# brodbeck-m/dolfinx_eqlb

Hardware: AMD Instinct MI355X
Metric: equilibrated patches/s (fp64) on 1M-tri Poisson k=2; L2 flux-divergence residual (higher is better)
Workload: dtype f64; 1 GPU; Poisson 1000000 triangles per GPU (crossed unit square 500x500), P2 primal, FluxEqlbSE RT2, homogeneous Dirichlet, fp64; headline=True, patches_per_gpu=501001, cells_per_gpu=1000000, nrhs=1, weak_symmetry=False, partition=none, solver=shuffle, scatter=tiled, accumulate=True

## Files before the change

dolfinx_eqlb_amd/csrc/eqlb_device_common.h:

```cpp
#pragma once

#include "eqlb_internal.h"

namespace eqlb
{

__host__ __device__ constexpr int nd_of(int deg) { return (deg + 1) * (deg + 2) / 2; }
__host__ __device__ constexpr int nrt_of(int k) { return k * (k + 2); }
__host__ __device__ constexpr int nq_of(int k) { return k * (k + 1) / 2; }
__host__ __device__ constexpr int binom(int n, int r)
{
  int v = 1;
  for (int i = 0; i < r; ++i)
    v = v * (n - i) / (i + 1);
  return v;
}
__host__ __device__ constexpr double bcoef(int j, int i)
{
  return (i > j) ? 0.0 : ((i % 2 == 0) ? 1.0 : -1.0) * binom(j, i);
}

#ifndef EQLB_WS_PIVOT_RTOL
#define EQLB_WS_PIVOT_RTOL 1e-11
#endif

__device__ __forceinline__ void wave_sync()
{
  __builtin_amdgcn_fence(__ATOMIC_RELEASE, "wavefront");
  __builtin_amdgcn_wave_barrier();
  __builtin_amdgcn_fence(__ATOMIC_ACQUIRE, "wavefront");
}

__device__ __forceinline__ double shfl_d(double v, int src_lane) { return __shfl(v, src_lane, 64); }

__device__ __forceinline__ int tri(int i, int j) { return i * (i + 1) / 2 + j; }

#ifndef EQLB_USE_DPP
#define EQLB_USE_DPP 1
#endif
template <int CTRL>
__device__ __forceinline__ double dpp_d(double v)
{
  int lo = __double2loint(v), hi = __double2hiint(v);
  lo = __builtin_amdgcn_update_dpp(0, lo, CTRL, 0xf, 0xf, true);
  hi = __builtin_amdgcn_update_dpp(0, hi, CTRL, 0xf, 0xf, true);
  return __hiloint2double(hi, lo);
}
template <int P, int OFF>
__device__ __forceinline__ double lane_down_d(double v, int gbase, int sub)
{
  if constexpr (EQLB_USE_DPP && P <= 16)
    return dpp_d<0x110 + OFF>(v);
  else if constexpr (EQLB_USE_DPP && OFF == 1)
    return dpp_d<0x138>(v);
  else
    return __shfl(v, gbase + ((sub >= OFF) ? sub - OFF : sub), 64);
}
template <int P>
__device__ __forceinline__ double lane_up1_d(double v, int gbase, int sub)
{
  if constexpr (EQLB_USE_DPP && P <= 16)
    return dpp_d<0x101>(v);
  else if constexpr (EQLB_USE_DPP)
    return dpp_d<0x130>(v);
  else
    return __shfl(v, gbase + ((sub + 1 < P) ? sub + 1 : sub), 64);
}
#ifndef EQLB_GSUM_SWIZZLE
#define EQLB_GSUM_SWIZZLE 0
#endif
template <int XOR>
__device__ __forceinline__ double swizzle_xor_d(double v)
{
  constexpr int PAT = (XOR << 10) | 0x1f;
  int lo = __double2loint(v), hi = __double2hiint(v);
  lo = __builtin_amdgcn_ds_swizzle(lo, PAT);
  hi = __builtin_amdgcn_ds_swizzle(hi, PAT);
  return __hiloint2double(hi, lo);
}
template <int P>
__device__ __forceinline__ double group_sum_d(double v, int gbase, int sub)
{
  if constexpr (EQLB_GSUM_SWIZZLE && P <= 16)
  {
    v += swizzle_xor_d<1>(v);
    v += swizzle_xor_d<2>(v);
    if constexpr (P >= 8)
      v += swizzle_xor_d<4>(v);
    if constexpr (P >= 16)
      v += swizzle_xor_d<8>(v);
    return v;
  }
  else if constexpr (EQLB_USE_DPP && P <= 16)
  {
    v += dpp_d<0xB1>(v);
    v += dpp_d<0x4E>(v);
    if constexpr (P >= 8)
      v += dpp_d<0x141>(v);
    if constexpr (P >= 16)
      v += dpp_d<0x140>(v);
    return v;
  }
  else
  {
#pragma unroll
    for (int off = 1; off < P; off <<= 1)
      v += __shfl(v, gbase + (sub ^ off), 64);
    return v;
  }
}

#ifndef EQLB_FAST_RCP
#define EQLB_FAST_RCP 1
#endif
__device__ __forceinline__ double rcp_d(double x)
{
#if EQLB_FAST_RCP
  double r = __builtin_amdgcn_rcp(x);
  r = __builtin_fma(__builtin_fma(-x, r, 1.0), r, r);
  r = __builtin_fma(__builtin_fma(-x, r, 1.0), r, r);
  return r;
#else
  return 1.0 / x;
#endif
}
__device__ __forceinline__ double rsqrt_d(double x)
{
#if EQLB_FAST_RCP
  double y = __builtin_amdgcn_rsq(x);
  y = __builtin_fma(y * 0.5, __builtin_fma(-x * y, y, 1.0), y);
  y = __builtin_fma(y * 0.5, __builtin_fma(-x * y, y, 1.0), y);
  return y;
#else
  return 1.0 / sqrt(x);
#endif
}


constexpr int NCOMBO = 12;
__host__ __device__ constexpr int combo_index(int fm, int fp, bool rev)
{
  return (fm * 2 + ((fp < fm) ? fp : fp - 1)) * 2 + (rev ? 1 : 0);
}

#ifndef EQLB_WQ_PAD
#define EQLB_WQ_PAD 0
#endif
template <int K, int DEG, int P>
struct Sizes
{
  static constexpr int KB = K - 1;
  static constexpr int NADD = (K - 1) * (K - 2) / 2;
  static constexpr int NDIV = K * (K + 1) / 2 - 1;
  static constexpr int NRT = nrt_of(K), ND = nd_of(DEG), NQ = nq_of(K);
  static constexpr int NY = 2 * K + NADD;
  static constexpr int NCOL = 2 * K + NDIV;
  static constexpr int NH = 1 + 2 * KB + NADD;
  static constexpr int NTE = NH * (NH + 1) / 2;
  static constexpr int NTES = NTE + (NTE & 1), NCOLS = NCOL + (NCOL & 1);
  static constexpr int DIMMAX = 1 + KB * P + NADD * P;
  static constexpr int TRI = DIMMAX * (DIMMAX + 1) / 2;
  static constexpr int LDS_GROUP = TRI + DIMMAX;
  static constexpr int HROW = ND * NQ + ((ND * NQ) & 1);
  static constexpr int NS = 3 * NRT * NRT, NF = 9 * ND * K, NHT = 3 * HROW, NDT = 6 * ND * NQ;
  static constexpr int NTET = NCOMBO * 3 * NTES, NWQT = NCOMBO * 3 * NH * NCOLS;
  static constexpr int NHB = 9 * K * K;
  static constexpr int NTAB = NF + NHT + NDT + NTET + NWQT + NHB;
  static constexpr int NVT = 3 * NRT * 2, NVQT = NCOMBO * 2 * NH * 3;
  static constexpr int OFF_TE = NS + NF + NHT + NDT, OFF_V = OFF_TE + NTET + NWQT + NHB, OFF_VQ = OFF_V + NVT;
  static constexpr int NHG = HROW, NWG = NCOMBO * NH * ND * 2, NEV = NHG + NWG;
  static constexpr int OFF_HG = OFF_VQ + NVQT;
  static constexpr int NCMB = 3 * NH * NCOLS, NCMBH = NCMB + ((K == 3) ? EQLB_WQ_PAD : 0);
  static constexpr int NWQH = (NCOMBO / 2) * NCMBH, NTAB_HALF = NTAB - NWQT + NWQH;
  static constexpr int NEV_LDS = (K >= 4) ? NHG : NEV;
  static constexpr int lds_doubles(int block, int solver, int mode = 0)
  {
    return NTAB + (mode ? NEV_LDS : 0) + ((K > 1 && solver == 0) ? (block / P) * LDS_GROUP : 0);
  }
  static constexpr int block_of(int solver)
  {
    if (K >= 4 && solver != 0 && P < 32)
      return 256;
    return (P >= 32) ? 64
                     : ((lds_doubles(256, solver) * 8 <= 65536)
                            ? 256
                            : ((lds_doubles(128, solver) * 8 <= 65536) ? 128 : 64));
  }
};


}
```

dolfinx_eqlb_amd/csrc/eqlb_se_kernels.hip:

```cpp
#include "eqlb_device_common.h"
#include "eqlb_tables_gen.h"

#ifndef EQLB_PCR_SELECTS
#define EQLB_PCR_SELECTS 0
#endif

#ifndef EQLB_SE_TEMPLATES_ONLY
#define EQLB_SE_TEMPLATES_ONLY 0
#endif

namespace eqlb
{

#if !EQLB_SE_TEMPLATES_ONLY
size_t table_doubles(int k, int deg)
{
  const int nrt = nrt_of(k), nd = nd_of(deg), nq = nq_of(k);
  const int kb = k - 1, nadd = (k - 1) * (k - 2) / 2, ndiv = k * (k + 1) / 2 - 1;
  const int nh = 1 + 2 * kb + nadd, ncol = 2 * k + ndiv;
  const int hrow = nd * nq + ((nd * nq) & 1);
  const int nte = nh * (nh + 1) / 2;
  return (size_t)3 * nrt * nrt + (size_t)9 * nd * k + (size_t)3 * hrow + (size_t)6 * nd * nq
         + (size_t)NCOMBO * 3 * (nte + (nte & 1)) + (size_t)NCOMBO * 3 * nh * (ncol + (ncol & 1))
         + (size_t)9 * k * k + (size_t)3 * nrt * 2 + (size_t)NCOMBO * 2 * nh * 3
// ... 52 lines not shown
  if (k == 1 && deg == 0)
    fill_tables_t<1, 0>(out);
  else if (k == 2 && deg == 1)
    fill_tables_t<2, 1>(out);
  else if (k == 3 && deg == 2)
    fill_tables_t<3, 2>(out);
  else if (k == 4 && deg == 3)
    fill_tables_t<4, 3>(out);
  else if (k == 2 && deg == 0)
    fill_tables_t<2, 0>(out);
  else if (k == 3 && deg == 1)
    fill_tables_t<3, 1>(out);
  else if (k == 3 && deg == 0)
    fill_tables_t<3, 0>(out);
  else if (k == 4 && deg >= 0 && deg < 3)
  {
    if (fill_tables_k4_lowdeg(deg, out) != 0)
      return EQLB_ERR_UNSUPPORTED;
  }
  else
    return EQLB_ERR_UNSUPPORTED;
  return (out.size() == table_doubles(k, deg)) ? 0 : EQLB_ERR_UNSUPPORTED;
}
#endif

#ifndef EQLB_EV_FMA
#define EQLB_EV_FMA 1
#endif
#ifndef EQLB_LE_FMA
#define EQLB_LE_FMA 1
#endif
#ifndef EQLB_P2_DIV_NODAL
#define EQLB_P2_DIV_NODAL 1
#endif
#ifndef EQLB_CHAIN_PCR
#define EQLB_CHAIN_PCR 1
#endif

template <bool AL>
__device__ __forceinline__ const double* row16(const double* p)
{
  if constexpr (AL)
    return static_cast<const double*>(__builtin_assume_aligned(p, 16));
  else
    return p;
}

template <int N>
__device__ __forceinline__ void ldrow16(const double* p, double (&r)[N])
{
  static_assert(N % 2 == 0, "row length");
  const double2* q = reinterpret_cast<const double2*>(p);
#pragma unroll
  for (int i = 0; i < N / 2; ++i)
  {
    const double2 v = q[i];
    r[2 * i] = v.x;
    r[2 * i + 1] = v.y;
  }
}

#ifndef EQLB_REV_FMA
#define EQLB_REV_FMA 1
#endif
template <int K>
__device__ __forceinline__ void reversal_apply(const double (&x)[K], const double rho, double (&y)[K])
{
#pragma unroll
  for (int j = 0; j < K; ++j)
  {
    double d = 0.0;
    bool any = false;
#pragma unroll
    for (int c = 0; c <= j; ++c)
    {
      const double coef = bcoef(j, c) - ((j == c) ? 1.0 : 0.0);
      if (coef != 0.0)
      {
        d = any ? __builtin_fma(coef, x[c], d) : coef * x[c];
        any = true;
      }
    }
    y[j] = any ? __builtin_fma(rho, d, x[j]) : x[j];
  }
}
template <int K>
__device__ __forceinline__ void reversal_apply_t(const double (&x)[K], const double rho, double (&y)[K])
{
#pragma unroll
  for (int h = 0; h < K; ++h)
  {
    double d = 0.0;
    bool any = false;
#pragma unroll
    for (int j = h; j < K; ++j)
    {
      const double coef = bcoef(j, h) - ((j == h) ? 1.0 : 0.0);
      if (coef != 0.0)
      {
        d = any ? __builtin_fma(coef, x[j], d) : coef * x[j];
        any = true;
      }
    }
    y[h] = any ? __builtin_fma(rho, d, x[h]) : x[h];
  }
}

template <int K, int DEG, int P, int SOLVER, int SCATTER, int BLOCK, int MODE = 0, bool FULL = false, bool INTR = false>
__device__ __forceinline__ void se_patch_body(const SeArgs& a, const int64_t block_id, double* lds,
                                              const bool tables_staged = false,
                                              const int64_t lane_index = -1, double* tile_slots = nullptr)
{
  using Z = Sizes<K, DEG, P>;
  constexpr int KB = Z::KB, NADD = Z::NADD, NDIV = Z::NDIV, NRT = Z::NRT, ND = Z::ND, NQ = Z::NQ;
  constexpr int NCOL = Z::NCOL, NH = Z::NH;

  constexpr bool AL = K == 2 && DEG == 1;
  static_assert(!AL || (Z::NF % 2 == 0 && Z::NHT % 2 == 0 && Z::NDT % 2 == 0 && Z::NTET % 2 == 0
                        && Z::NWQT % 2 == 0 && (ND * K) % 2 == 0 && Z::HROW % 2 == 0
                        && Z::NTES % 2 == 0 && Z::NCOLS % 2 == 0 && Z::NHB % 2 == 0
                        && Z::NHG % 2 == 0),
                "table rows are not 16-byte aligned");
  double* sF = lds;
  double* sH = sF + Z::NF;
  double* sD = sH + Z::NHT;
  double* sTE = sD + Z::NDT;
  constexpr bool HALFWQ = SCATTER == 2 && K == 3;
  double* sWQ = sTE + Z::NTET;
  double* sHB = sWQ + (HALFWQ ? Z::NWQH : Z::NWQT);
  double* sHG = sHB + Z::NHB;
  const double* sWG = (K >= 4) ? a.tables + Z::OFF_HG + Z::NHG : sHG + Z::NHG;
  (void)sWG;
  double* sA = sHB + Z::NHB + (MODE ? Z::NEV_LDS : 0);
  (void)sA;

  int tid_ = threadIdx.x;
#ifndef EQLB_OPAQUE_K3
#define EQLB_OPAQUE_K3 1
#endif
  if constexpr (SCATTER == 2 && (MODE == 1 || (EQLB_OPAQUE_K3 && K >= 3)))
    asm volatile("" : "+v"(tid_));
  const int tid = tid_;
  if (!tables_staged)
  {
    for (int i = tid; i < Z::NTAB; i += BLOCK)
      lds[i] = a.tables[Z::NS + i];
    if constexpr (MODE == 1)
      for (int i = tid; i < Z::NEV_LDS; i += BLOCK)
        sHG[i] = a.tables[Z::OFF_HG + i];
    __syncthreads();
  }

  const int lane = tid & 63;
  const int sub = lane % P;
  const int gbase = lane - sub;
  const int64_t tl = (lane_index >= 0) ? lane_index : block_id * BLOCK + tid;
  const int64_t patch_local = tl / P;
#ifndef EQLB_FULL_SIMPLE
#define EQLB_FULL_SIMPLE 1
#endif
#ifndef EQLB_FULL_SIMPLE_EV
#define EQLB_FULL_SIMPLE_EV 0
#endif
  constexpr bool FULLS = FULL && EQLB_FULL_SIMPLE && (MODE == 0 || K >= 3 || EQLB_FULL_SIMPLE_EV);
  const bool pvalid = FULLS ? true : (patch_local < a.npatch);
  const int64_t slot = a.slot_offset + tl;
  const int64_t patch = a.patch_offset + patch_local;

  const int r = a.rhs;
  int n = 0;
  int32_t cell_raw = -1;
  uint32_t info = 0u;
  uint8_t flag0 = (uint8_t)PFLAG_INTERIOR, flag = (uint8_t)0;
  if (pvalid)
  {
    n = (int)a.pn[patch];
    cell_raw = a.slot_cell[slot];
    info = a.slot_info[slot];
    flag0 = a.pflag[patch];
    flag = a.pflag[(int64_t)r * a.npatch_total + patch];
  }
  if constexpr (FULL)
  {
    n = P;
    flag0 = (uint8_t)PFLAG_INTERIOR;
    flag = (uint8_t)0;
  }
  if constexpr (INTR)
  {
    flag0 = (uint8_t)PFLAG_INTERIOR;
    flag = (uint8_t)0;
  }
  const bool active = FULL ? true : (cell_raw >= 0);
  const int32_t cell = active ? cell_raw : 0;
  const int fm = (info >> INFO_FM_SHIFT) & 3, fp = (info >> INFO_FP_SHIFT) & 3;
  const int ln = (info >> INFO_LN_SHIFT) & 3;
  const bool rev_m = (info & INFO_REV_M) != 0, rev_p = (info & INFO_REV_P) != 0;
  const int ci = active ? combo_index(fm, fp, rev_m) : 0;
  const double rho_m = rev_m ? 1.0 : 0.0, rho_p = rev_p ? 1.0 : 0.0;
  (void)rho_m;
  (void)rho_p;

  double J00 = 1.0, J01 = 0.0, J10 = 0.0, J11 = 1.0;
  double2 gdat[ND];
  double fdat[ND];
#pragma unroll
  for (int i = 0; i < ND; ++i)
  {
    gdat[i] = make_double2(0.0, 0.0);
    fdat[i] = 0.0;
  }
  if (active)
  {
    const double2* Jp = reinterpret_cast<const double2*>(a.cellJ + 4 * (int64_t)cell);
    const double2* gp_ = reinterpret_cast<const double2*>(a.flux_dg + ((int64_t)a.rhs_in * a.ncells + cell) * (ND * 2));
    const double* fp_ = a.rhs_dg + ((int64_t)a.rhs_in * a.ncells + cell) * ND;
    const double2 j0 = Jp[0], j1 = Jp[1];
#pragma unroll
    for (int i = 0; i < ND; ++i)
      gdat[i] = gp_[i];
#pragma unroll
    for (int i = 0; i < ND; ++i)
      fdat[i] = fp_[i];
    J00 = j0.x;
    J01 = j0.y;
    J10 = j1.x;
    J11 = j1.y;
  }
  const double detJ = J00 * J11 - J01 * J10;
  const double sgn = (detJ > 0.0) ? 1.0 : -1.0;
  const double pf_m = (fm == 1) ? sgn : -sgn;
  const double pf_p = (fp == 1) ? sgn : -sgn;

  const bool interior_geo = (flag0 & PFLAG_INTERIOR) != 0;
  const int nf = interior_geo ? n : n + 1;
  const int nn = (n > 0) ? n : 1;
  const int next = FULLS ? ((sub + 1) & (P - 1)) : ((sub + 1 < nn) ? sub + 1 : (interior_geo ? 0 : sub));
  const int prev = FULLS ? ((sub + P - 1) & (P - 1)) : ((sub > 0) ? sub - 1 : (interior_geo ? nn - 1 : 0));
  const bool has_next = active && (interior_geo || sub < n - 1);
  const bool has_prev = active && (interior_geo || sub > 0);
  const int fi_p = FULLS ? next : (interior_geo ? ((sub + 1 < nn) ? sub + 1 : 0) : sub + 1);
  const int dim = pvalid ? 1 + KB * nf + NADD * n : 0;
  (void)dim;

  int status_local = 0;

  {
    const bool bc0 = (flag & PFLAG_BC0) != 0, bcn = (flag & PFLAG_BCN) != 0;
    const bool d_fixed = bc0 || bcn;

    double gm[K], gpv[K], Rq[NQ];
    double LeG[MODE ? NH : 1];
    (void)LeG;
    {
      const double a00 = J11, a01 = -J01, a10 = -J10, a11 = J00;
      const double nmx = (fm == 2) ? 0.0 : -1.0, nmy = (fm == 0) ? -1.0 : ((fm == 1) ? 0.0 : 1.0);
      const double npx = (fp == 2) ? 0.0 : -1.0, npy = (fp == 0) ? -1.0 : ((fp == 1) ? 0.0 : 1.0);
      const double num0 = a00 * nmx + a10 * nmy, num1 = a01 * nmx + a11 * nmy;
      const double nup0 = a00 * npx + a10 * npy, nup1 = a01 * npx + a11 * npy;
#pragma unroll
      for (int j = 0; j < K; ++j)
        gm[j] = gpv[j] = 0.0;
#pragma unroll
      for (int q = 0; q < NQ; ++q)
        Rq[q] = 0.0;
      if constexpr (MODE == 1)
      {
#pragma unroll
        for (int h = 0; h < NH; ++h)
          LeG[h] = 0.0;
        if (active)
        {
          const double* tH = row16<AL>(sH + ln * Z::HROW);
          const double* wg = row16<AL>(sWG + ci * NH * ND * 2);

          const double dh0 = (ln == 0) ? -1.0 : ((ln == 1) ? 1.0 : 0.0);
          const double dh1 = (ln == 0) ? -1.0 : ((ln == 2) ? 1.0 : 0.0);
#pragma unroll
          for (int i = 0; i < ND; ++i)
          {
            const double2 g2 = gdat[i];
            const double fd = detJ * fdat[i];
            const double gg = dh0 * (a00 * g2.x + a01 * g2.y) + dh1 * (a10 * g2.x + a11 * g2.y);
            const double jt0 = J00 * g2.x + J10 * g2.y, jt1 = J01 * g2.x + J11 * g2.y;
#pragma unroll
            for (int q = 0; q < NQ; ++q)
#if EQLB_EV_FMA
              Rq[q] = __builtin_fma(gg, sHG[i * NQ + q], __builtin_fma(fd, tH[i * NQ + q], Rq[q]));
#else
              Rq[q] += fd * tH[i * NQ + q] + gg * sHG[i * NQ + q];
#endif
#pragma unroll
            for (int h = 0; h < NH; ++h)
            {
              if constexpr (AL)
              {
                const double2 w2 = reinterpret_cast<const double2*>(wg)[h * ND + i];
#if EQLB_EV_FMA
                LeG[h] = __builtin_fma(w2.y, jt1, __builtin_fma(w2.x, jt0, LeG[h]));
#else
                LeG[h] += w2.x * jt0 + w2.y * jt1;
#endif
              }
              else
#if EQLB_EV_FMA
                LeG[h] = __builtin_fma(wg[(h * ND + i) * 2 + 1], jt1, __builtin_fma(wg[(h * ND + i) * 2], jt0, LeG[h]));
#else
                LeG[h] += wg[(h * ND + i) * 2] * jt0 + wg[(h * ND + i) * 2 + 1] * jt1;
#endif
            }
          }
        }
      }
      else if (active)
      {
        const double* tF_m = row16<AL>(sF + (fm * 3 + ln) * ND * K);
        const double* tF_p = row16<AL>(sF + (fp * 3 + ln) * ND * K);
        const double* tH = row16<AL>(sH + ln * Z::HROW);
        const double* tD = sD + ln * ND * 2 * NQ;
        double fdv[ND], dvg = 0.0;
        double ax[(DEG == 2) ? ND : 1], by[(DEG == 2) ? ND : 1];
        (void)fdv;
        (void)tD;
        (void)ax;
        (void)by;
#pragma unroll
        for (int i = 0; i < ND; ++i)
        {
          const double2 g2 = gdat[i];
          const double fv = fdat[i];
          const double gnm = g2.x * num0 + g2.y * num1;
          const double gnp = g2.x * nup0 + g2.y * nup1;
          const double gh0 = a00 * g2.x + a01 * g2.y;
          const double gh1 = a10 * g2.x + a11 * g2.y;
          const double fd = detJ * fv;
          if constexpr (AL)
          {
            double rm[K], rp[K];
            ldrow16<K>(tF_m + i * K, rm);
            ldrow16<K>(tF_p + i * K, rp);
#pragma unroll
            for (int j = 0; j < K; ++j)
            {
              gm[j] += rm[j] * gnm;
              gpv[j] += rp[j] * gnp;
            }
          }
          else
          {
#pragma unroll
            for (int j = 0; j < K; ++j)
            {
              gm[j] += tF_m[i * K + j] * gnm;
              gpv[j] += tF_p[i * K + j] * gnp;
            }
          }
          if constexpr (DEG == 1)
          {
            fdv[i] = fd;
            if (i == 0)
              dvg = -(gh0 + gh1);
            else if (i == 1)
              dvg += gh0;
            else
              dvg += gh1;
          }
          else if constexpr (DEG == 0 && K >= 2)
          {
#pragma unroll
            for (int q = 0; q < NQ; ++q)
              Rq[q] = __builtin_fma(fd, tH[q], Rq[q]);
          }
          else if constexpr (DEG == 2 && EQLB_P2_DIV_NODAL)
          {
            fdv[i] = fd;
            ax[i] = gh0;
            by[i] = gh1;
          }
          else
          {
#pragma unroll
            for (int q = 0; q < NQ; ++q)
              Rq[q] = __builtin_fma(-gh1, tD[(i * 2 + 1) * NQ + q],
                                    __builtin_fma(-gh0, tD[(i * 2 + 0) * NQ + q], __builtin_fma(fd, tH[i * NQ + q], Rq[q])));
          }
        }
        if constexpr (DEG == 2 && EQLB_P2_DIV_NODAL)
        {
          double dvn[ND];
          dvn[0] = 4.0 * (ax[5] + by[4]) - 3.0 * (ax[0] + by[0]) - ax[1] - by[2];
          dvn[1] = ax[0] + by[0] + 3.0 * ax[1] - by[2] + 4.0 * (by[3] - by[5] - ax[5]);
          dvn[2] = ax[0] + by[0] - ax[1] + 3.0 * by[2] + 4.0 * (ax[3] - ax[4] - by[4]);
          dvn[3] = 0.5 * (dvn[1] + dvn[2]);
          dvn[4] = 0.5 * (dvn[0] + dvn[2]);
          dvn[5] = 0.5 * (dvn[0] + dvn[1]);
#pragma unroll
          for (int i = 0; i < ND; ++i)
          {
            const double w = fdv[i] - dvn[i];
#pragma unroll
            for (int q = 0; q < NQ; ++q)
              Rq[q] = __builtin_fma(w, tH[i * NQ + q], Rq[q]);
          }
        }
        if constexpr (DEG == 1)
        {
          double rH[Z::HROW];
          if constexpr (AL)
            ldrow16<Z::HROW>(tH, rH);
          else
          {
#pragma unroll
            for (int e = 0; e < ND * NQ; ++e)
              rH[e] = tH[e];
          }
#pragma unroll
          for (int i = 0; i < ND; ++i)
#pragma unroll
            for (int q = 0; q < NQ; ++q)
              Rq[q] += (fdv[i] - dvg) * rH[i * NQ + q];
        }
#pragma unroll
        for (int j = 0; j < K; ++j)
        {
          gm[j] *= pf_m;
          gpv[j] *= pf_p;
        }
      }
    }

    double mu_m[K], mu_p[K];
    {
      double Jv[K];
      {
        double gmn[K];
#pragma unroll
        for (int j = 0; j < K; ++j)
          gmn[j] = shfl_d(gm[j], gbase + next);
#if EQLB_REV_FMA
        double gt[K];
        reversal_apply<K>(gmn, rho_p, gt);
#pragma unroll
        for (int j = 0; j < K; ++j)
          Jv[j] = has_next ? gpv[j] + gt[j] : 0.0;
#else
#pragma unroll
        for (int j = 0; j < K; ++j)
        {
          double t = 0.0;
          if (rev_p)
          {
#pragma unroll
            for (int i = 0; i < K; ++i)
              t += bcoef(j, i) * gmn[i];
          }
          else
            t = gmn[j];
          Jv[j] = has_next ? gpv[j] + t : 0.0;
        }
#endif
      }
      const double Jprev0 = shfl_d(Jv[0], gbase + prev);
      double t = active ? (sgn * Rq[0] + (has_prev ? Jprev0 : 0.0)) : 0.0;
      {
        double o = lane_down_d<P, 1>(t, gbase, sub);
        if (sub >= 1)
          t += o;
        if constexpr (P > 2)
        {
          o = lane_down_d<P, 2>(t, gbase, sub);
          if (sub >= 2)
            t += o;
        }
        if constexpr (P > 4)
        {
          o = lane_down_d<P, 4>(t, gbase, sub);
          if (sub >= 4)
            t += o;
        }
        if constexpr (P > 8)
        {
          o = lane_down_d<P, 8>(t, gbase, sub);
          if (sub >= 8)
            t += o;
        }
#pragma unroll
        for (int off = 16; off < P; off <<= 1)
        {
          o = shfl_d(t, gbase + ((sub >= off) ? sub - off : sub));
          if (sub >= off)
            t += o;
        }
      }
      double bnd_m[K], bnd_p[K];
#pragma unroll
      for (int j = 0; j < K; ++j)
      {
        bnd_m[j] = -gm[j];
        bnd_p[j] = -gpv[j];
      }
      if (a.bvals != nullptr && active && d_fixed)
      {
        const bool at0 = bc0 && sub == 0, atn = bcn && sub == n - 1;
        if (at0 || atn)
        {
          const double* bv = a.bvals + ((int64_t)r * a.ncells + cell) * NRT;
#pragma unroll
          for (int side = 0; side < 2; ++side)
          {
            if (!(side == 0 ? at0 : atn))
              continue;
            const int fb = side == 0 ? fm : fp;
            const double pfb = side == 0 ? pf_m : pf_p;
            double bg[K];
            bool allzero = true;
#pragma unroll
            for (int j = 0; j < K; ++j)
            {
              bg[j] = bv[fb * K + j];
              allzero = allzero && (fabs(bg[j]) < 1e-7);
            }
            if (!allzero)
            {
              const double* hb = sHB + (fb * 3 + ln) * K * K;
#pragma unroll
              for (int i = 0; i < K; ++i)
              {
                double s = 0.0;
#pragma unroll
                for (int j = 0; j < K; ++j)
                  s += hb[i * K + j] * bg[j];
                if (side == 0)
                  bnd_m[i] += pfb * s;
                else
                  bnd_p[i] += pfb * s;
              }
            }
          }
        }
      }
      double delta = 0.0;
      if (d_fixed)
      {
        const double m0_first = shfl_d(bnd_m[0], gbase);
        const double p0_last = shfl_d(bnd_p[0], gbase + nn - 1);
        const double t_last = shfl_d(t, gbase + nn - 1);
        delta = bc0 ? -m0_first : (p0_last - t_last);
      }
      mu_p[0] = t + delta;
#pragma unroll
      for (int j = 1; j < K; ++j)
        mu_p[j] = (bcn && sub == n - 1) ? bnd_p[j] : 0.0;
      double vprev[K];
#pragma unroll
      for (int j = 0; j < K; ++j)
        vprev[j] = shfl_d(mu_p[j] + Jv[j], gbase + prev);
      if (has_prev)
      {
#if EQLB_REV_FMA
        double vt[K];
        reversal_apply<K>(vprev, rho_m, vt);
#pragma unroll
        for (int j = 0; j < K; ++j)
          mu_m[j] = -vt[j];
#else
#pragma unroll
        for (int j = 0; j < K; ++j)
        {
          double s = 0.0;
#pragma unroll
          for (int c = 0; c < K; ++c)
            s -= (rev_m ? bcoef(j, c) : ((j == c) ? 1.0 : 0.0)) * vprev[c];
          mu_m[j] = s;
        }
#endif
      }
      else
      {
        mu_m[0] = -delta;
#pragma unroll
        for (int j = 1; j < K; ++j)
          mu_m[j] = bc0 ? bnd_m[j] : 0.0;
      }
    }

    double Te[NH][NH], Le[NH];
    {
      const double ia = active ? rcp_d(fabs(detJ)) : 0.0;
      const double g0 = (J00 * J00 + J10 * J10) * ia, g1 = (J00 * J01 + J10 * J11) * ia,
                   g2 = (J01 * J01 + J11 * J11) * ia;
      constexpr int NTES = Z::NTES, NCOLS = Z::NCOLS;
      const double* te = row16<AL>(sTE + ci * 3 * NTES);
      if constexpr (AL)
      {
        double tev[NTES];
#pragma unroll
        for (int e2 = 0; e2 < NTES / 2; ++e2)
        {
          const double2 t0 = reinterpret_cast<const double2*>(te)[e2];
          const double2 t1 = reinterpret_cast<const double2*>(te + NTES)[e2];
          const double2 t2 = reinterpret_cast<const double2*>(te + 2 * NTES)[e2];
          tev[2 * e2] = g0 * t0.x + g1 * t1.x + g2 * t2.x;
          tev[2 * e2 + 1] = g0 * t0.y + g1 * t1.y + g2 * t2.y;
        }
#pragma unroll
        for (int h = 0; h < NH; ++h)
#pragma unroll
          for (int g = 0; g <= h; ++g)
          {
            const double v = tev[h * (h + 1) / 2 + g];
            Te[h][g] = v;
            Te[g][h] = v;
          }
      }
      else
      {
#pragma unroll
        for (int h = 0; h < NH; ++h)
#pragma unroll
          for (int g = 0; g <= h; ++g)
          {
            const int e = h * (h + 1) / 2 + g;
            const double v = g0 * te[e] + g1 * te[NTES + e] + g2 * te[2 * NTES + e];
            Te[h][g] = v;
            Te[g][h] = v;
          }
      }
      double full[NCOL];
#pragma unroll
      for (int j = 0; j < K; ++j)
      {
        full[j] = mu_m[j];
        full[K + j] = mu_p[j];
      }
#pragma unroll
      for (int q = 0; q < NDIV; ++q)
        full[2 * K + q] = sgn * Rq[1 + q];
      const double* wq = row16<AL>(sWQ + (HALFWQ ? (ci >> 1) * Z::NCMBH : ci * 3 * NH * NCOLS));
#pragma unroll
      for (int h = 0; h < NH; ++h)
      {
        double s0 = 0.0, s1 = 0.0, s2 = 0.0;
        if constexpr (AL)
        {
#pragma unroll
          for (int c2 = 0; c2 < NCOLS / 2; ++c2)
          {
            const double2 w0 = reinterpret_cast<const double2*>(wq + h * NCOLS)[c2];
            const double2 w1 = reinterpret_cast<const double2*>(wq + (NH + h) * NCOLS)[c2];
            const double2 w2 = reinterpret_cast<const double2*>(wq + (2 * NH + h) * NCOLS)[c2];
            const double f0 = full[2 * c2], f1 = (2 * c2 + 1 < NCOL) ? full[2 * c2 + 1] : 0.0;
#if EQLB_LE_FMA
            s0 = __builtin_fma(w0.y, f1, __builtin_fma(w0.x, f0, s0));
            s1 = __builtin_fma(w1.y, f1, __builtin_fma(w1.x, f0, s1));
            s2 = __builtin_fma(w2.y, f1, __builtin_fma(w2.x, f0, s2));
#else
            s0 += w0.x * f0 + w0.y * f1;
            s1 += w1.x * f0 + w1.y * f1;
            s2 += w2.x * f0 + w2.y * f1;
#endif
          }
        }
        else
        {
#pragma unroll
          for (int c = 0; c < NCOL; ++c)
          {
            s0 += wq[h * NCOLS + c] * full[c];
            s1 += wq[(NH + h) * NCOLS + c] * full[c];
            s2 += wq[(2 * NH + h) * NCOLS + c] * full[c];
          }
        }
        Le[h] = -(g0 * s0 + g1 * s1 + g2 * s2);
      }
      if constexpr (HALFWQ)
      {
        double lt[K];
#if EQLB_REV_FMA
        double lk[K];
#pragma unroll
        for (int h = 0; h < K; ++h)
          lk[h] = Le[h];
        reversal_apply_t<K>(lk, rho_m, lt);
#pragma unroll
        for (int h = 0; h < K; ++h)
          Le[h] = lt[h];
#else
#pragma unroll
        for (int h = 0; h < K; ++h)
        {
          double t = 0.0;
#pragma unroll
          for (int j = h; j < K; ++j)
            t += bcoef(j, h) * Le[j];
          lt[h] = t;
        }
#pragma unroll
        for (int h = 0; h < K; ++h)
          Le[h] = rev_m ? lt[h] : Le[h];
#endif
      }
      if constexpr (MODE == 1)
      {
#pragma unroll
        for (int h = 0; h < NH; ++h)
          Le[h] += LeG[h];
      }
    }

// ... 168 lines not shown
      static_assert(NADD <= 3, "interior-DOF condensation is written for at most three DOFs per cell (k <= 4)");
      constexpr int W = K;
      constexpr int NC = 1 + 2 * KB;
      const bool fx_m = (bc0 && sub == 0) || (bcn && sub == n);
      const bool fx_p = bcn && sub == n - 1;
      const int prevl = FULLS ? prev : ((sub > 0) ? sub - 1 : nn - 1);
      const bool has_prevcell = pvalid && sub < nf && (sub > 0 || interior_geo);

      double(&T)[NH][NH] = Te;
      double(&Lv)[NH] = Le;
      if (d_fixed || fx_m || fx_p)
      {
#pragma unroll
        for (int h = 0; h < NH; ++h)
        {
          const bool fh = (h == 0) ? d_fixed : ((h <= KB) ? fx_m : ((h <= 2 * KB) ? fx_p : false));
          if (fh)
            Lv[h] = 0.0;
#pragma unroll
          for (int g = 0; g < NH; ++g)
          {
            const bool fg = (g == 0) ? d_fixed : ((g <= KB) ? fx_m : ((g <= 2 * KB) ? fx_p : false));
            if (fh || fg)
              T[h][g] = 0.0;
          }
        }
      }
      constexpr int NA1 = (NADD > 0) ? NADD : 1;
      double ca[NC][NA1], la[NA1];
#pragma unroll
      for (int h = 0; h < NC; ++h)
#pragma unroll
        for (int q = 0; q < NA1; ++q)
          ca[h][q] = 0.0;
#pragma unroll
      for (int q = 0; q < NA1; ++q)
        la[q] = 0.0;
      if constexpr (NADD == 1)
      {
        const double piv = active ? T[NC][NC] : 1.0;
        const double ip = rcp_d(piv);
        la[0] = Lv[NC] * ip;
#pragma unroll
        for (int h = 0; h < NC; ++h)
          ca[h][0] = T[h][NC] * ip;
#pragma unroll
        for (int h = 0; h < NC; ++h)
        {
          Lv[h] -= T[h][NC] * la[0];
#pragma unroll
          for (int g = 0; g <= h; ++g)
          {
            const double v = T[h][g] - ca[h][0] * T[NC][g];
            T[h][g] = v;
            T[g][h] = v;
          }
        }
      }
      else if constexpr (NADD > 1)
      {
        double Li[NADD][NADD], iLd[NADD], Inv[NADD][NADD];
#pragma unroll
        for (int i = 0; i < NADD; ++i)
#pragma unroll
          for (int j = 0; j <= i; ++j)
            Li[i][j] = active ? T[NC + i][NC + j] : ((i == j) ? 1.0 : 0.0);
#pragma unroll
        for (int j = 0; j < NADD; ++j)
        {
          double dj = Li[j][j];
#pragma unroll
          for (int q = 0; q < j; ++q)
            dj -= Li[j][q] * Li[j][q];
          if (!(dj > 0.0))
          {
            status_local = pvalid ? 1 : status_local;
            dj = 1.0;
          }
          const double ilj = rsqrt_d(dj);
          Li[j][j] = dj * ilj;
          iLd[j] = ilj;
#pragma unroll
          for (int i = j + 1; i < NADD; ++i)
          {
            double v = Li[i][j];
#pragma unroll
            for (int q = 0; q < j; ++q)
              v -= Li[i][q] * Li[j][q];
            Li[i][j] = v * ilj;
          }
        }
#pragma unroll
        for (int c = 0; c < NADD; ++c)
        {
          double y[NADD];
#pragma unroll
          for (int i = 0; i < NADD; ++i)
          {
            double v = (i == c) ? 1.0 : 0.0;
#pragma unroll
            for (int q = 0; q < i; ++q)
              v -= Li[i][q] * y[q];
            y[i] = v * iLd[i];
          }
#pragma unroll
          for (int i = NADD - 1; i >= 0; --i)
          {
            double v = y[i];
#pragma unroll
            for (int q = i + 1; q < NADD; ++q)
              v -= Li[q][i] * Inv[q][c];
            Inv[i][c] = v * iLd[i];
          }
        }
#pragma unroll
        for (int q = 0; q < NADD; ++q)
        {
          double v = 0.0;
#pragma unroll
          for (int q2 = 0; q2 < NADD; ++q2)
            v += Inv[q][q2] * Lv[NC + q2];
          la[q] = v;
        }
#pragma unroll
        for (int h = 0; h < NC; ++h)
#pragma unroll
          for (int q = 0; q < NADD; ++q)
          {
            double v = 0.0;
#pragma unroll
            for (int q2 = 0; q2 < NADD; ++q2)
              v += T[h][NC + q2] * Inv[q2][q];
            ca[h][q] = v;
          }
#pragma unroll
        for (int h = 0; h < NC; ++h)
        {
#pragma unroll
          for (int q = 0; q < NADD; ++q)
            Lv[h] -= T[h][NC + q] * la[q];
#pragma unroll
          for (int g = 0; g <= h; ++g)
          {
            double v = T[h][g];
#pragma unroll
            for (int q = 0; q < NADD; ++q)
              v -= ca[h][q] * T[NC + q][g];
            T[h][g] = v;
            T[g][h] = v;
          }
        }
      }
      double Dg[KB][KB], bt[KB], rr[KB], Off[KB][KB];
      double alpha = group_sum_d<P>(T[0][0], gbase, sub), rd = group_sum_d<P>(Lv[0], gbase, sub);
      if (d_fixed || !pvalid)
      {
        alpha = 1.0;
        rd = 0.0;
      }
#pragma unroll
      for (int aa = 0; aa < KB; ++aa)
      {
        const double dp_prev = shfl_d(T[0][1 + KB + aa], gbase + prevl);
        const double lp_prev = shfl_d(Lv[1 + KB + aa], gbase + prevl);
        bt[aa] = T[0][1 + aa] + (has_prevcell ? dp_prev : 0.0);
        rr[aa] = Lv[1 + aa] + (has_prevcell ? lp_prev : 0.0);
#pragma unroll
        for (int bb = 0; bb < KB; ++bb)
        {
          const double pp_prev = shfl_d(T[1 + KB + aa][1 + KB + bb], gbase + prevl);
          Dg[aa][bb] = T[1 + aa][1 + bb] + (has_prevcell ? pp_prev : 0.0);
          Off[aa][bb] = T[1 + aa][1 + KB + bb];
        }
      }
      const bool row_valid = pvalid && sub < nf && !fx_m;
      if (!row_valid)
      {
#pragma unroll
        for (int aa = 0; aa < KB; ++aa)
        {
          bt[aa] = rr[aa] = 0.0;
#pragma unroll
          for (int bb = 0; bb < KB; ++bb)
          {
            Dg[aa][bb] = (aa == bb) ? 1.0 : 0.0;
            Off[aa][bb] = 0.0;
          }
        }
      }
      double Z[W][W], rz[W], Off0[KB][KB];
      Z[0][0] = alpha;
      rz[0] = rd;
#pragma unroll
      for (int aa = 0; aa < KB; ++aa)
      {
        const double b0 = shfl_d(bt[aa], gbase);
        Z[0][1 + aa] = Z[1 + aa][0] = b0;
        rz[1 + aa] = shfl_d(rr[aa], gbase);
#pragma unroll
        for (int bb = 0; bb < KB; ++bb)
        {
          Z[1 + aa][1 + bb] = shfl_d(Dg[aa][bb], gbase);
          Off0[aa][bb] = shfl_d(Off[aa][bb], gbase);
        }
      }
      const bool in_chain = pvalid && sub >= 1 && sub < nf;
      const bool wraps = interior_geo && sub == n - 1;
      double Dp[KB][KB], Rp[KB][1 + W], OffC[KB][KB];
#ifndef EQLB_CHAIN_MASKS
#define EQLB_CHAIN_MASKS 1
#endif
      if constexpr (FULLS && EQLB_CHAIN_MASKS && KB >= 2)
      {
        const double mc = (sub >= 1) ? 1.0 : 0.0, mi = 1.0 - mc;
        const double mo = (sub >= 1 && sub != P - 1) ? 1.0 : 0.0;
        const double m1 = (sub == 1) ? 1.0 : 0.0, mw = mc - mo;
#pragma unroll
        for (int aa = 0; aa < KB; ++aa)
        {
          Rp[aa][0] = mc * rr[aa];
          Rp[aa][1] = mc * bt[aa];
#pragma unroll
          for (int bb = 0; bb < KB; ++bb)
          {
            Dp[aa][bb] = (aa == bb) ? __builtin_fma(mc, Dg[aa][bb], mi) : mc * Dg[aa][bb];
            OffC[aa][bb] = mo * Off[aa][bb];
            Rp[aa][2 + bb] = __builtin_fma(mw, Off[aa][bb], m1 * Off0[bb][aa]);
          }
        }
      }
      else
      {
#pragma unroll
      for (int aa = 0; aa < KB; ++aa)
      {
        Rp[aa][0] = in_chain ? rr[aa] : 0.0;
        Rp[aa][1] = in_chain ? bt[aa] : 0.0;
#pragma unroll
        for (int bb = 0; bb < KB; ++bb)
        {
          Dp[aa][bb] = in_chain ? Dg[aa][bb] : ((aa == bb) ? 1.0 : 0.0);
          OffC[aa][bb] = (in_chain && !wraps) ? Off[aa][bb] : 0.0;
          double c0 = 0.0;
          if (in_chain && sub == 1)
            c0 += Off0[bb][aa];
          if (in_chain && wraps)
            c0 += Off[aa][bb];
          Rp[aa][2 + bb] = c0;
        }
      }
      }
      double zz[W], xs[KB];
      if constexpr (KB == 1 && P <= 16 && EQLB_CHAIN_PCR)
      {
        double b = Dp[0][0], r0 = Rp[0][0], r1 = Rp[0][1], r2 = Rp[0][2];
        const double B1 = Rp[0][1], B2 = Rp[0][2];
        double am = dpp_d<0x111>(OffC[0][0]);
        if (!(FULLS && EQLB_CHAIN_MASKS) && sub == 0)
          am = 0.0;
        bool posdef = true;
#define EQLB_PCR_LEVEL(S)                                                                          \
  if constexpr (P > S)                                                                             \
  {                                                                                                \
    posdef = posdef && (b > 0.0);                                                                  \
    const double ib = rcp_d(b);                                                                    \
    const double ib_lo = dpp_d<0x110 + S>(ib), a_lo = dpp_d<0x110 + S>(am);                        \
    const double r0_lo = dpp_d<0x110 + S>(r0), r1_lo = dpp_d<0x110 + S>(r1), r2_lo = dpp_d<0x110 + S>(r2); \
    const double ib_hi = dpp_d<0x100 + S>(ib), a_hi = dpp_d<0x100 + S>(am);                        \
    const double r0_hi = dpp_d<0x100 + S>(r0), r1_hi = dpp_d<0x100 + S>(r1), r2_hi = dpp_d<0x100 + S>(r2); \
    const double cp = EQLB_PCR_SELECTS ? ((sub + S < P) ? a_hi : 0.0) : a_hi;  \
    const double al = am * ib_lo, ga = cp * ib_hi;                                                 \
    b = __builtin_fma(-ga, cp, __builtin_fma(-al, am, b));                                         \
    r0 = __builtin_fma(-ga, r0_hi, __builtin_fma(-al, r0_lo, r0));                                 \
    r1 = __builtin_fma(-ga, r1_hi, __builtin_fma(-al, r1_lo, r1));                                 \
    r2 = __builtin_fma(-ga, r2_hi, __builtin_fma(-al, r2_lo, r2));                                 \
    am = EQLB_PCR_SELECTS ? ((sub >= 2 * S) ? -al * a_lo : 0.0) : -al * a_lo;                      \
  }
        EQLB_PCR_LEVEL(1)
        EQLB_PCR_LEVEL(2)
        EQLB_PCR_LEVEL(4)
        EQLB_PCR_LEVEL(8)
#undef EQLB_PCR_LEVEL
        posdef = posdef && (b > 0.0);
        const double ibf = rcp_d(b);
        const double s0 = r0 * ibf, s1 = r1 * ibf, s2 = r2 * ibf;
        double tred[W], Sred[W][W];
        tred[0] = group_sum_d<P>(B1 * s0, gbase, sub);
        tred[1] = group_sum_d<P>(B2 * s0, gbase, sub);
        Sred[0][0] = group_sum_d<P>(B1 * s1, gbase, sub);
        Sred[1][0] = group_sum_d<P>(B2 * s1, gbase, sub);
        Sred[1][1] = group_sum_d<P>(B2 * s2, gbase, sub);
        {
          const double l00 = Z[0][0] - Sred[0][0], l10 = Z[1][0] - Sred[1][0];
          const double i0 = rcp_d(l00);
          const double m = l10 * i0;
          const double d1 = __builtin_fma(-m, l10, Z[1][1] - Sred[1][1]);
          posdef = posdef && (l00 > 0.0) && (d1 > 0.0);
          const double q0 = rz[0] - tred[0];
          const double q1 = __builtin_fma(-m, q0, rz[1] - tred[1]);
          zz[1] = q1 * rcp_d(d1);
          zz[0] = __builtin_fma(-l10, zz[1], q0) * i0;
        }
        if (!posdef && pvalid)
          status_local = 1;
        const double v = __builtin_fma(-s2, zz[1], __builtin_fma(-s1, zz[0], s0));
        xs[0] = in_chain ? v : 0.0;
      }
      else
      {
        double Ei[KB][KB], X[KB][1 + W], Y[KB][KB];
        auto finish_row = [&]() {
          if constexpr (KB == 1)
            Ei[0][0] = rcp_d(Dp[0][0]);
          else if constexpr (KB == 3)
          {
            const double c00 = Dp[1][1] * Dp[2][2] - Dp[1][2] * Dp[2][1];
            const double c01 = Dp[0][2] * Dp[2][1] - Dp[0][1] * Dp[2][2];
            const double c02 = Dp[0][1] * Dp[1][2] - Dp[0][2] * Dp[1][1];
            const double c11 = Dp[0][0] * Dp[2][2] - Dp[0][2] * Dp[2][0];
            const double c12 = Dp[0][2] * Dp[1][0] - Dp[0][0] * Dp[1][2];
            const double c22 = Dp[0][0] * Dp[1][1] - Dp[0][1] * Dp[1][0];
            const double det = Dp[0][0] * c00 + Dp[0][1] * c01 + Dp[0][2] * c02;
            const double id = rcp_d(det);
            Ei[0][0] = c00 * id;
            Ei[0][1] = Ei[1][0] = c01 * id;
            Ei[0][2] = Ei[2][0] = c02 * id;
            Ei[1][1] = c11 * id;
            Ei[1][2] = Ei[2][1] = c12 * id;
            Ei[2][2] = c22 * id;
          }
          else
          {
            const double det = Dp[0][0] * Dp[1][1] - Dp[0][1] * Dp[1][0];
            const double id = rcp_d(det);
            Ei[0][0] = Dp[1][1] * id;
            Ei[1][1] = Dp[0][0] * id;
            Ei[0][1] = -Dp[0][1] * id;
            Ei[1][0] = -Dp[1][0] * id;
          }
  #pragma unroll
          for (int aa = 0; aa < KB; ++aa)
          {
// ... 144 lines not shown
              {
                double v = 0.0;
    #pragma unroll
                for (int e = 0; e < KB; ++e)
                  v += OffC[e][aa] * X[e][c];
                P2[aa][c] = v;
              }
            }
            const bool take = in_chain && sub == s;
    #pragma unroll
            for (int aa = 0; aa < KB; ++aa)
            {
    #pragma unroll
              for (int bb = 0; bb < KB; ++bb)
              {
                const double v = lane_down_d<P, 1>(P1[aa][bb], gbase, sub);
                if (take)
                  Dp[aa][bb] -= v;
              }
    #pragma unroll
              for (int c = 0; c < 1 + W; ++c)
              {
                const double v = lane_down_d<P, 1>(P2[aa][c], gbase, sub);
                if (take)
                  Rp[aa][c] -= v;
              }
            }
          }
          finish_row();
        }
        double Sred[W][W], tred[W];
  #pragma unroll
        for (int c = 0; c < W; ++c)
        {
          double v = 0.0;
  #pragma unroll
          for (int e = 0; e < KB; ++e)
            v += Rp[e][1 + c] * X[e][0];
          tred[c] = v;
  #pragma unroll
          for (int c2 = 0; c2 <= c; ++c2)
          {
            double u2 = 0.0;
  #pragma unroll
            for (int e = 0; e < KB; ++e)
              u2 += Rp[e][1 + c] * X[e][1 + c2];
            Sred[c][c2] = u2;
          }
        }
  #pragma unroll
        for (int c = 0; c < W; ++c)
        {
          tred[c] = group_sum_d<P>(tred[c], gbase, sub);
  #pragma unroll
          for (int c2 = 0; c2 <= c; ++c2)
            Sred[c][c2] = group_sum_d<P>(Sred[c][c2], gbase, sub);
        }
          {
          double Lz[W][W], iLz[W];
  #pragma unroll
          for (int c = 0; c < W; ++c)
          {
            rz[c] -= tred[c];
  #pragma unroll
            for (int c2 = 0; c2 <= c; ++c2)
              Lz[c][c2] = Z[c][c2] - Sred[c][c2];
          }
  #pragma unroll
          for (int j = 0; j < W; ++j)
          {
            double dj = Lz[j][j];
  #pragma unroll
            for (int q = 0; q < j; ++q)
              dj -= Lz[j][q] * Lz[j][q];
            if (!(dj > 0.0))
            {
              status_local = pvalid ? 1 : status_local;
              dj = 1.0;
            }
            const double ilj = rsqrt_d(dj), lj = dj * ilj;
            Lz[j][j] = lj;
            iLz[j] = ilj;
  #pragma unroll
            for (int i = j + 1; i < W; ++i)
            {
              double v = Lz[i][j];
  #pragma unroll
              for (int q = 0; q < j; ++q)
                v -= Lz[i][q] * Lz[j][q];
              Lz[i][j] = v * ilj;
            }
          }
  #pragma unroll
          for (int i = 0; i < W; ++i)
          {
            double v = rz[i];
  #pragma unroll
            for (int q = 0; q < i; ++q)
              v -= Lz[i][q] * zz[q];
            zz[i] = v * iLz[i];
          }
  #pragma unroll
          for (int i = W - 1; i >= 0; --i)
          {
            double v = zz[i];
  #pragma unroll
            for (int q = i + 1; q < W; ++q)
              v -= Lz[q][i] * zz[q];
            zz[i] = v * iLz[i];
          }
        }
  #pragma unroll
        for (int aa = 0; aa < KB; ++aa)
        {
          double v = X[aa][0];
  #pragma unroll
          for (int c = 0; c < W; ++c)
            v -= X[aa][1 + c] * zz[c];
          xs[aa] = in_chain ? v : 0.0;
        }
  #ifdef EQLB_EXP_CHAIN3
        constexpr int SBACK = (P == 8 || P == 16) ? 0 : P - 2;
  #else
        constexpr int SBACK = P - 2;
  #endif
  #pragma unroll 1
        for (int s = BLOCK_PCR ? 0 : SBACK; s >= 1; --s)
        {
          double xn[KB];
  #pragma unroll
          for (int aa = 0; aa < KB; ++aa)
            xn[aa] = lane_up1_d<P>(xs[aa], gbase, sub);
          if (in_chain && sub == s)
          {
  #pragma unroll
            for (int aa = 0; aa < KB; ++aa)
  #pragma unroll
              for (int bb = 0; bb < KB; ++bb)
                xs[aa] -= Y[aa][bb] * xn[bb];
          }
        }
      }
#pragma unroll
      for (int aa = 0; aa < KB; ++aa)
        if (sub == 0)
          xs[aa] = zz[1 + aa];
      ul[0] = zz[0];
#pragma unroll
      for (int aa = 0; aa < KB; ++aa)
      {
        ul[1 + aa] = xs[aa];
        ul[1 + KB + aa] = shfl_d(xs[aa], gbase + ((fi_p < P) ? fi_p : 0));
      }
      if constexpr (NADD >= 1)
      {
#pragma unroll
        for (int q = 0; q < NADD; ++q)
        {
          double v = la[q];
#pragma unroll
          for (int h = 0; h < NC; ++h)
            v -= ca[h][q] * ul[h];
          ul[NC + q] = v;
        }
      }
      if (!active)
      {
#pragma unroll
        for (int h = 0; h < NH; ++h)
          ul[h] = 0.0;
      }
    }


    if (active)
    {
      double ym[K], yp[K];
#if EQLB_REV_FMA
      double uk[K], ut[K];
#pragma unroll
      for (int c = 0; c < K; ++c)
        uk[c] = ul[c];
      reversal_apply<K>(uk, rho_m, ut);
#pragma unroll
      for (int j = 0; j < K; ++j)
      {
        ym[j] = mu_m[j] - ut[j];
        yp[j] = mu_p[j] + ((j == 0) ? ul[0] : ul[KB + j]);
      }
#else
#pragma unroll
      for (int j = 0; j < K; ++j)
      {
        double s = mu_m[j];
#pragma unroll
        for (int c = 0; c < K; ++c)
          s -= (rev_m ? bcoef(j, c) : ((j == c) ? 1.0 : 0.0)) * ul[c];
        ym[j] = s;
        yp[j] = mu_p[j] + ((j == 0) ? ul[0] : ul[KB + j]);
      }
#endif
      if constexpr (SCATTER == 2)
      {
        const uint32_t loc = info >> INFO_LOCAL_SHIFT;
#ifdef EQLB_EXP_NOSTORE
        if (loc != 0u)
          tile_slots[loc] = ym[0] + yp[0] + ym[K - 1] + yp[K - 1] + Rq[NQ - 1] + ul[NH - 1];
        else
#endif
        if (loc != 0u)
        {
          constexpr int NPK = NRT - K;
          double* o = tile_slots + ((int64_t)(loc - 1) * 3 + ln) * NPK;
          const int pm = fm - ((fm > ln) ? 1 : 0), pp = fp - ((fp > ln) ? 1 : 0);
#pragma unroll
          for (int j = 0; j < K; ++j)
          {
            o[pm * K + j] = pf_m * ym[j];
            o[pp * K + j] = pf_p * yp[j];
          }
#pragma unroll
          for (int q = 0; q < NDIV; ++q)
            o[2 * K + q] = Rq[1 + q];
#pragma unroll
          for (int q = 0; q < NADD; ++q)
            o[2 * K + NDIV + q] = sgn * ul[1 + 2 * KB + q];
        }
      }
      double cout[(SCATTER == 2) ? 1 : NRT];
      if constexpr (SCATTER != 2)
      {
#pragma unroll
        for (int e = 0; e < 3 * K; ++e)
        {
          const int fe = e / K, j = e % K;
          cout[e] = (fe == fm) ? pf_m * ym[j] : ((fe == fp) ? pf_p * yp[j] : 0.0);
        }
#pragma unroll
        for (int q = 0; q < NDIV; ++q)
          cout[3 * K + q] = Rq[1 + q];
#pragma unroll
        for (int q = 0; q < NADD; ++q)
          cout[3 * K + NDIV + q] = sgn * ul[1 + 2 * KB + q];
      }
      (void)cout;
      if constexpr (SCATTER == 2)
      {
      }
      else if constexpr (SCATTER == 0)
      {
#ifdef EQLB_EXP_SLOTROW
        double* o = a.out + (slot % ((int64_t)a.ncells * 3)) * NRT;
#else
        double* o = a.out + (((int64_t)a.rhs_out * a.ncells + cell) * 3 + ln) * NRT;
#endif
#pragma unroll
        for (int e = 0; e < NRT; ++e)
          o[e] = cout[e];
      }
      else
      {
        double* o = a.out + ((int64_t)a.rhs_out * a.ncells + cell) * NRT;
#pragma unroll
        for (int e = 0; e < NRT; ++e)
          unsafeAtomicAdd(o + e, cout[e]);
      }
    }
  }

  if (status_local)
    atomicOr(a.status, 1);
}

#ifndef EQLB_K4_WAVES
#define EQLB_K4_WAVES 1
#endif
template <int K, int DEG, int P, int SOLVER, int SCATTER, int MODE = 0>
__global__ void __launch_bounds__((Sizes<K, DEG, P>::block_of(SOLVER)), ((K >= 4 && SOLVER == 1) ? EQLB_K4_WAVES : 1))
k_se_patch(const SeArgs a)
{
  extern __shared__ __align__(16) double lds[];
  se_patch_body<K, DEG, P, SOLVER, SCATTER, Sizes<K, DEG, P>::block_of(SOLVER), MODE>(a, blockIdx.x, lds);
}

template <int K, int DEG, int SOLVER, int SCATTER>
#ifndef EQLB_FUSED_WAVES
#define EQLB_FUSED_WAVES 4
#endif
#ifndef EQLB_PERSIST_OVERSUB
#define EQLB_PERSIST_OVERSUB 1
#endif
__global__ void __launch_bounds__(256, (K <= 2 ? EQLB_FUSED_WAVES : 1)) k_se_patch_fused(const SeArgs a0, const FusedBins fb)
{
  extern __shared__ __align__(16) double lds[];
  using Z = Sizes<K, DEG, 8>;
  for (int i = threadIdx.x; i < Z::NTAB; i += 256)
    lds[i] = a0.tables[Z::NS + i];
  __syncthreads();
  const int64_t nwork = fb.block_start[MAX_BINS];
  for (int64_t bid = blockIdx.x; bid < nwork; bid += gridDim.x)
  {
    int b = 0;
#pragma unroll
    for (int i = 1; i < MAX_BINS; ++i)
      if (bid >= fb.block_start[i])
        b = i;
// ... 856 lines not shown
```

Measured before the change: 6.365 billion patches/s.

## Add ring-mapped DPP lane layout with cyclic reduction for K=2 patch solve

```diff
diff --git a/dolfinx_eqlb_amd/csrc/eqlb_device_common.h b/dolfinx_eqlb_amd/csrc/eqlb_device_common.h
--- a/dolfinx_eqlb_amd/csrc/eqlb_device_common.h
+++ b/dolfinx_eqlb_amd/csrc/eqlb_device_common.h
@@ -108,6 +108,35 @@
       v += __shfl(v, gbase + (sub ^ off), 64);
     return v;
   }
+}
+
+template <int P, int S>
+__device__ __forceinline__ double ring_prev_d(double v)
+{
+  static_assert((P == 4 || P == 8) && S >= 1 && S < P, "ring lane map: P = 4, 8");
+  return dpp_d<0x120 + (16 / P) * S>(v);
+}
+template <int P, int S>
+__device__ __forceinline__ double ring_next_d(double v)
+{
+  static_assert((P == 4 || P == 8) && S >= 1 && S < P, "ring lane map: P = 4, 8");
+  return dpp_d<0x120 + 16 - (16 / P) * S>(v);
+}
+template <int P, int OFF>
+__device__ __forceinline__ double ring_down_d(double v)
+{
+  static_assert((P == 4 || P == 8) && OFF >= 1 && OFF < P, "ring lane map: P = 4, 8");
+  return dpp_d<0x110 + (16 / P) * OFF>(v);
+}
+template <int P>
+__device__ __forceinline__ double ring_sum_d(double v)
+{
+  static_assert(P == 4 || P == 8, "ring lane map: P = 4, 8");
+  if constexpr (P == 8)
+    v += dpp_d<0x4E>(v);
+  v += dpp_d<0x128>(v);
+  v += dpp_d<0x124>(v);
+  return v;
 }
 
 #ifndef EQLB_FAST_RCP
diff --git a/dolfinx_eqlb_amd/csrc/eqlb_se_kernels.hip b/dolfinx_eqlb_amd/csrc/eqlb_se_kernels.hip
--- a/dolfinx_eqlb_amd/csrc/eqlb_se_kernels.hip
+++ b/dolfinx_eqlb_amd/csrc/eqlb_se_kernels.hip
@@ -228,10 +228,6 @@
   }
 
   const int lane = tid & 63;
-  const int sub = lane % P;
-  const int gbase = lane - sub;
-  const int64_t tl = (lane_index >= 0) ? lane_index : block_id * BLOCK + tid;
-  const int64_t patch_local = tl / P;
 #ifndef EQLB_FULL_SIMPLE
 #define EQLB_FULL_SIMPLE 1
 #endif
@@ -239,6 +235,18 @@
 #define EQLB_FULL_SIMPLE_EV 0
 #endif
   constexpr bool FULLS = FULL && EQLB_FULL_SIMPLE && (MODE == 0 || K >= 3 || EQLB_FULL_SIMPLE_EV);
+#ifndef EQLB_RING_PCR
+#define EQLB_RING_PCR 1
+#endif
+  constexpr bool RING = EQLB_RING_PCR && FULLS && K == 2 && MODE == 0 && SOLVER == 1 && SCATTER == 2 && (P == 4 || P == 8)
+                        && EQLB_USE_DPP && EQLB_CHAIN_PCR;
+  constexpr int RP = RING ? P : 4;
+  constexpr int RQ = RING ? 16 / P : 1;
+  const int sub = RING ? (lane & 15) / RQ : lane % P;
+  const int gbase = RING ? (lane & ~15) : lane - sub;
+  const int64_t tl = RING ? lane_index - (lane & 15) + ((lane & 15) % RQ) * P + sub
+                          : ((lane_index >= 0) ? lane_index : block_id * BLOCK + tid);
+  const int64_t patch_local = tl / P;
   const bool pvalid = FULLS ? true : (patch_local < a.npatch);
   const int64_t slot = a.slot_offset + tl;
   const int64_t patch = a.patch_offset + patch_local;
@@ -512,7 +520,7 @@
         double gmn[K];
 #pragma unroll
         for (int j = 0; j < K; ++j)
-          gmn[j] = shfl_d(gm[j], gbase + next);
+          gmn[j] = RING ? ring_next_d<RP, 1>(gm[j]) : shfl_d(gm[j], gbase + next);
 #if EQLB_REV_FMA
         double gt[K];
         reversal_apply<K>(gmn, rho_p, gt);
@@ -536,8 +544,24 @@
         }
 #endif
       }
-      const double Jprev0 = shfl_d(Jv[0], gbase + prev);
+      const double Jprev0 = RING ? ring_prev_d<RP, 1>(Jv[0]) : shfl_d(Jv[0], gbase + prev);
       double t = active ? (sgn * Rq[0] + (has_prev ? Jprev0 : 0.0)) : 0.0;
+      if constexpr (RING)
+      {
+        double o = ring_down_d<RP, 1>(t);
+        if (sub >= 1)
+          t += o;
+        o = ring_down_d<RP, 2>(t);
+        if (sub >= 2)
+          t += o;
+        if constexpr (P > 4)
+        {
+          o = ring_down_d<RP, 4>(t);
+          if (sub >= 4)
+            t += o;
+        }
+      }
+      else
       {
         double o = lane_down_d<P, 1>(t, gbase, sub);
         if (sub >= 1)
@@ -630,7 +654,7 @@
       double vprev[K];
 #pragma unroll
       for (int j = 0; j < K; ++j)
-        vprev[j] = shfl_d(mu_p[j] + Jv[j], gbase + prev);
+        vprev[j] = RING ? ring_prev_d<RP, 1>(mu_p[j] + Jv[j]) : shfl_d(mu_p[j] + Jv[j], gbase + prev);
       if (has_prev)
       {
 #if EQLB_REV_FMA
@@ -1105,7 +1129,8 @@
         }
       }
       double Dg[KB][KB], bt[KB], rr[KB], Off[KB][KB];
-      double alpha = group_sum_d<P>(T[0][0], gbase, sub), rd = group_sum_d<P>(Lv[0], gbase, sub);
+      double alpha = RING ? ring_sum_d<RP>(T[0][0]) : group_sum_d<P>(T[0][0], gbase, sub);
+      double rd = RING ? ring_sum_d<RP>(Lv[0]) : group_sum_d<P>(Lv[0], gbase, sub);
       if (d_fixed || !pvalid)
       {
         alpha = 1.0;
@@ -1114,14 +1139,15 @@
 #pragma unroll
       for (int aa = 0; aa < KB; ++aa)
       {
-        const double dp_prev = shfl_d(T[0][1 + KB + aa], gbase + prevl);
-        const double lp_prev = shfl_d(Lv[1 + KB + aa], gbase + prevl);
+        const double dp_prev = RING ? ring_prev_d<RP, 1>(T[0][1 + KB + aa]) : shfl_d(T[0][1 + KB + aa], gbase + prevl);
+        const double lp_prev = RING ? ring_prev_d<RP, 1>(Lv[1 + KB + aa]) : shfl_d(Lv[1 + KB + aa], gbase + prevl);
         bt[aa] = T[0][1 + aa] + (has_prevcell ? dp_prev : 0.0);
         rr[aa] = Lv[1 + aa] + (has_prevcell ? lp_prev : 0.0);
 #pragma unroll
         for (int bb = 0; bb < KB; ++bb)
         {
-          const double pp_prev = shfl_d(T[1 + KB + aa][1 + KB + bb], gbase + prevl);
+          const double pp_prev = RING ? ring_prev_d<RP, 1>(T[1 + KB + aa][1 + KB + bb])
+                                      : shfl_d(T[1 + KB + aa][1 + KB + bb], gbase + prevl);
           Dg[aa][bb] = T[1 + aa][1 + bb] + (has_prevcell ? pp_prev : 0.0);
           Off[aa][bb] = T[1 + aa][1 + KB + bb];
         }
@@ -1141,6 +1167,52 @@
           }
         }
       }
+      if constexpr (RING)
+      {
+        double b = Dg[0][0], r0 = rr[0], r1 = bt[0];
+        double am = ring_prev_d<RP, 1>(Off[0][0]);
+        bool posdef = true;
+#define EQLB_RING_LEVEL(S)                                                                         \
+  if constexpr (P >= 4 * S)                                                                        \
+  {                                                                                                \
+    posdef = posdef && (b > 0.0);                                                                  \
+    const double ib = rcp_d(b);                                                                    \
+    const double ib_lo = ring_prev_d<RP, S>(ib), a_lo = ring_prev_d<RP, S>(am);                    \
+    const double r0_lo = ring_prev_d<RP, S>(r0), r1_lo = ring_prev_d<RP, S>(r1);                   \
+    const double ib_hi = ring_next_d<RP, S>(ib), a_hi = ring_next_d<RP, S>(am);                    \
+    const double r0_hi = ring_next_d<RP, S>(r0), r1_hi = ring_next_d<RP, S>(r1);                   \
+    const double al = am * ib_lo, ga = a_hi * ib_hi;                                               \
+    b = __builtin_fma(-ga, a_hi, __builtin_fma(-al, am, b));                                       \
+    r0 = __builtin_fma(-ga, r0_hi, __builtin_fma(-al, r0_lo, r0));                                 \
+    r1 = __builtin_fma(-ga, r1_hi, __builtin_fma(-al, r1_lo, r1));                                 \
+    am = -al * a_lo;                                                                               \
+  }
+        EQLB_RING_LEVEL(1)
+        EQLB_RING_LEVEL(2)
+#undef EQLB_RING_LEVEL
+        double s0, s1;
+        {
+          constexpr int H = RP / 2;
+          const double b_o = ring_prev_d<RP, H>(b), a_o = ring_prev_d<RP, H>(am);
+          const double r0_o = ring_prev_d<RP, H>(r0), r1_o = ring_prev_d<RP, H>(r1);
+          const double c = am + a_o;
+          const double det = __builtin_fma(b, b_o, -c * c);
+          posdef = posdef && (b > 0.0) && (det > 0.0);
+          const double id = rcp_d(det);
+          s0 = __builtin_fma(b_o, r0, -c * r0_o) * id;
+          s1 = __builtin_fma(b_o, r1, -c * r1_o) * id;
+        }
+        const double t0 = ring_sum_d<RP>(bt[0] * s0), t1 = ring_sum_d<RP>(bt[0] * s1);
+        const double piv = alpha - t1;
+        posdef = posdef && (piv > 0.0);
+        if (!posdef)
+          status_local = 1;
+        ul[0] = (rd - t0) * rcp_d(piv);
+        ul[1] = __builtin_fma(-s1, ul[0], s0);
+        ul[2] = ring_next_d<RP, 1>(ul[1]);
+      }
+      else
+      {
       double Z[W][W], rz[W], Off0[KB][KB];
       Z[0][0] = alpha;
       rz[0] = rd;
@@ -1591,6 +1663,7 @@
         ul[1 + aa] = xs[aa];
         ul[1 + KB + aa] = shfl_d(xs[aa], gbase + ((fi_p < P) ? fi_p : 0));
       }
+      }
       if constexpr (NADD >= 1)
       {
 #pragma unroll
```

Result: faster. 6.890 billion patches/s, median of 6 (+8.2%).
